# haotiansun14/rl-rep

Measured on NVIDIA B200. Metric: agent updates/sec, higher is better.
Workload: dtype tf32

## Files before the change

### rlrep_b200/csrc/gemm_chain.cu

```cuda
#include <algorithm>
#include <cmath>
#include <cstdlib>
#include <cstring>

#include "common.cuh"
#include "gemm_chain.cuh"
#include "ptx.cuh"

namespace rlrep {

namespace {

constexpr int kThreads = 320;
constexpr int kEpiWarps = 8;
constexpr int kStages = 6;
constexpr int kCW = 16;
constexpr int kTwPitch = kCW + 4;
constexpr int kMaxBn = 128;
constexpr int kBM = 128, kBK = 32;
constexpr int kABytes = kBM * kBK * 4;
constexpr int kStageBytes = kABytes + kMaxBn * kBK * 4;
constexpr int kTbufFloats = kEpiWarps * 32 * kTwPitch;
constexpr int kSub = 4, kCtrStride = 32;
constexpr int kDbgItems = 16, kDbgEvents = 10;
constexpr int kSmemBytes = kStages * kStageBytes + 1024 + 256 + kTbufFloats * 4;
static_assert(kSmemBytes <= 227 * 1024, "chain kernel shared memory");

__device__ __forceinline__ void red_release_add(unsigned* p, unsigned v) {
  asm volatile("red.release.gpu.global.add.u32 [%0], %1;" ::"l"(p), "r"(v) : "memory");
}
__device__ __forceinline__ unsigned atom_add_acq_rel(unsigned* p, unsigned v) {
  unsigned old;
  asm volatile("atom.acq_rel.gpu.global.add.u32 %0, [%1], %2;" : "=r"(old) : "l"(p), "r"(v) : "memory");
  return old;
}
__device__ __forceinline__ void fence_proxy_async_global() { asm volatile("fence.proxy.async.global;" ::: "memory"); }
__device__ __forceinline__ void fence_tensormap_acquire(const CUtensorMap* m) {
  asm volatile("fence.proxy.tensormap::generic.acquire.gpu [%0], 128;" ::"l"(reinterpret_cast<uint64_t>(m)) : "memory");
}
__device__ __forceinline__ unsigned ld_relaxed(const unsigned* p) {
  unsigned v;
  asm volatile("ld.relaxed.gpu.global.u32 %0, [%1];" : "=r"(v) : "l"(p) : "memory");
  return v;
}
__device__ __forceinline__ void wait_counter(const unsigned* done, int dep, int dep_tiles) {
  const unsigned* p = done + (size_t)dep * kSub * kCtrStride;
  unsigned target[kSub];
#pragma unroll
  for (int sub = 0; sub < kSub; ++sub) target[sub] = (unsigned)((dep_tiles - sub + kSub - 1) / kSub);
  long long t0 = 0;
  while (true) {
    unsigned v[kSub];
#pragma unroll
    for (int sub = 0; sub < kSub; ++sub) v[sub] = ld_relaxed(p + sub * kCtrStride);
    bool ok = true;
#pragma unroll
    for (int sub = 0; sub < kSub; ++sub) ok = ok && v[sub] >= target[sub];
    if (ok) return;
    __nanosleep(20);
    if (t0 == 0) t0 = clock64();
    if (clock64() - t0 > 4000000000LL) {
      printf("rlrep: chain dependency wait timed out (block %d, gemm %d, tiles %d, counters %u %u %u %u)\n", blockIdx.x, dep,
             dep_tiles, v[0], v[1], v[2], v[3]);
      __trap();
    }
  }
}
__device__ __forceinline__ void fence_acquire_gpu() { asm volatile("fence.acq_rel.gpu;" ::: "memory"); }

__device__ __forceinline__ void epilogue_bar() { asm volatile("bar.sync 1, 256;" ::: "memory"); }

__device__ __forceinline__ float elu_fast(float x) {
  const float n = fminf(x, 0.f);
  float p = 1.f / 5040.f;
  p = fmaf(p, n, 1.f / 720.f);
  p = fmaf(p, n, 1.f / 120.f);
  p = fmaf(p, n, 1.f / 24.f);
  p = fmaf(p, n, 1.f / 6.f);
  p = fmaf(p, n, 0.5f);
  p = fmaf(p, n, 1.f);
  p *= n;
  const float e = __expf(n) - 1.f;
  const float r = n < -0.34657359f ? e : p;
  return x > 0.f ? x : r;
}

__device__ __forceinline__ bool aligned16(const void* p) { return (reinterpret_cast<uintptr_t>(p) & 15) == 0; }

__device__ __forceinline__ float chain_epilogue_scalar(const Epilogue& e, float acc, int m, int n, const float* cptr) {
  float v = acc * e.scale;
  if (e.r1_u) v = fmaf(__ldcg(e.r1_u + m), __ldcg(e.r1_v + n), v);
  if (e.bias) v += __ldg(e.bias + n);
  if (e.pre_out) e.pre_out[(size_t)m * e.ld_pre + n] = v;
  v = apply_act(v, e.act);
  if (e.dact != DACT_NONE) v *= apply_dact(__ldcg(e.aux + (size_t)m * e.ld_aux + n), e.dact);
  if (e.accumulate) v += __ldcg(cptr);
  return v;
}

struct ChunkOperands {
  float4 bias, r1v;
  float4 aux[4];
  float r1u[4];
};
__device__ __forceinline__ void chunk_prefetch(ChunkOperands& o, const Epilogue& epi, int M, int m_base, int gn0, int lane) {
  const int piece = lane & 3, rsub = lane >> 2;
  const int on = gn0 + 4 * piece;
  o.bias = make_float4(0.f, 0.f, 0.f, 0.f);
  o.r1v = make_float4(0.f, 0.f, 0.f, 0.f);
  if (epi.bias) o.bias = __ldg(reinterpret_cast<const float4*>(epi.bias + on));
  if (epi.r1_u) o.r1v = __ldcg(reinterpret_cast<const float4*>(epi.r1_v + on));
#pragma unroll
  for (int r4 = 0; r4 < 4; ++r4) {
    const int om = m_base + r4 * 8 + rsub;
    o.aux[r4] = make_float4(0.f, 0.f, 0.f, 0.f);
    o.r1u[r4] = 0.f;
    if (om < M) {
      if (epi.dact != DACT_NONE) o.aux[r4] = __ldcg(reinterpret_cast<const float4*>(epi.aux + (size_t)om * epi.ld_aux + on));
      if (epi.r1_u) o.r1u[r4] = __ldcg(epi.r1_u + om);
    }
  }
}

template <int ACT, int DACT>
__device__ __forceinline__ void chain_store_rows(const Epilogue& epi, const ChunkOperands& o, const float* tw,
                                                 float* __restrict__ C, int ldc, int M, int m_base, int gn0, int lane) {
  const int piece = lane & 3, rsub = lane >> 2;
  const int on = gn0 + 4 * piece;
#pragma unroll
  for (int r4 = 0; r4 < 4; ++r4) {
    const int r = r4 * 8 + rsub;
    const int om = m_base + r;
    if (om < M) {
      const float4 a4 = *reinterpret_cast<const float4*>(tw + r * kTwPitch + 4 * piece);
      float v[4] = {a4.x * epi.scale, a4.y * epi.scale, a4.z * epi.scale, a4.w * epi.scale};
      if (epi.r1_u) {
        const float u = o.r1u[r4];
        v[0] = fmaf(u, o.r1v.x, v[0]); v[1] = fmaf(u, o.r1v.y, v[1]); v[2] = fmaf(u, o.r1v.z, v[2]); v[3] = fmaf(u, o.r1v.w, v[3]);
      }
      v[0] += o.bias.x; v[1] += o.bias.y; v[2] += o.bias.z; v[3] += o.bias.w;
      if (epi.pre_out)
        *reinterpret_cast<float4*>(epi.pre_out + (size_t)om * epi.ld_pre + on) = make_float4(v[0], v[1], v[2], v[3]);
      if constexpr (ACT != ACT_NONE) {
#pragma unroll
        for (int e = 0; e < 4; ++e) v[e] = ACT == ACT_ELU ? elu_fast(v[e]) : apply_act(v[e], ACT < 0 ? epi.act : ACT);
      }
      if constexpr (DACT != DACT_NONE) {
        const int dact = DACT < 0 ? epi.dact : DACT;
        if (dact != DACT_NONE) {
          const float4 x = o.aux[r4];
          v[0] *= apply_dact(x.x, dact); v[1] *= apply_dact(x.y, dact); v[2] *= apply_dact(x.z, dact); v[3] *= apply_dact(x.w, dact);
        }
      }
      float4* cp = reinterpret_cast<float4*>(C + (size_t)om * ldc + on);
      if (epi.accumulate) {
        const float4 c0 = __ldcg(cp);
        v[0] += c0.x; v[1] += c0.y; v[2] += c0.z; v[3] += c0.w;
      }
      *cp = make_float4(v[0], v[1], v[2], v[3]);
    }
  }
}

__global__ void __launch_bounds__(kThreads, 1)
gemm_chain_kernel(const ChainGemmDesc* __restrict__ gemms, const ChainTask* __restrict__ tasks,
                  const int* __restrict__ task_begin, unsigned* __restrict__ done, unsigned* __restrict__ exit_ctr,
                  int n_gemms, unsigned long long* __restrict__ dbg) {
  auto stamp = [&](int item, int ev) {
    if (dbg != nullptr && item < kDbgItems) {
      unsigned long long t;
      asm volatile("mov.u64 %0, %%globaltimer;" : "=l"(t)::"memory");
      dbg[((size_t)blockIdx.x * kDbgItems + item) * kDbgEvents + ev] = t;
    }
  };
  if (threadIdx.x == 0) stamp(kDbgItems - 1, 2);
  extern __shared__ uint8_t smem_raw[];
  uint8_t* smem = reinterpret_cast<uint8_t*>((reinterpret_cast<uintptr_t>(smem_raw) + 1023) & ~uintptr_t(1023));
  uint64_t* full_bar = reinterpret_cast<uint64_t*>(smem + kStages * kStageBytes);
  uint64_t* empty_bar = full_bar + 8;
  uint64_t* acc_full = empty_bar + 8;
  uint64_t* acc_empty = acc_full + 2;
  uint32_t* tmem_slot = reinterpret_cast<uint32_t*>(acc_empty + 2);
  volatile unsigned* arrival = reinterpret_cast<volatile unsigned*>(tmem_slot + 1);
  float* tbuf = reinterpret_cast<float*>(smem + kStages * kStageBytes + 256);

  const int warp = threadIdx.x >> 5, lane = threadIdx.x & 31;
  const int t_begin = task_begin[blockIdx.x], t_end = task_begin[blockIdx.x + 1];

  if (threadIdx.x == 0) {
    for (int s = 0; s < kStages; ++s) {
      ptx::mbar_init(&full_bar[s], 1);
      ptx::mbar_init(&empty_bar[s], 1);
    }
    for (int a = 0; a < 2; ++a) {
      ptx::mbar_init(&acc_full[a], 1);
      ptx::mbar_init(&acc_empty[a], kEpiWarps);
    }
    ptx::fence_mbar_init();
  }
  if (warp == 1) {
    ptx::tmem_alloc(tmem_slot, 2 * kMaxBn);
    ptx::tmem_relinquish();
  }
  ptx::tc_fence_before_sync();
  __syncthreads();
  ptx::tc_fence_after_sync();
  const uint32_t tmem_base = *tmem_slot;
  ptx::pdl_wait();

  if (warp == 0) {
    if (lane == 0) {
      int it = 0, last_gemm = -1;
      for (int t = t_begin; t < t_end; ++t) {
        const ChainTask tk = tasks[t];
        const ChainGemmDesc* g = gemms + tk.gemm;
        const int n_deps = g->n_deps;
        const int bn = g->bn, a_mn = g->a_mn, b_mn = g->b_mn;
        const int m0 = (tk.tile % g->tiles_m) * kBM, n0 = (tk.tile / g->tiles_m) * bn;
        const int kb0 = tk.split * g->kb_per_split, kb1 = min(g->nkb, kb0 + g->kb_per_split);
        int dep_id[kChainMaxDeps], dep_tiles[kChainMaxDeps];
#pragma unroll
        for (int d = 0; d < kChainMaxDeps; ++d) {
          dep_id[d] = d < n_deps ? g->dep[d] : 0;
          dep_tiles[d] = d < n_deps ? (int)g->dep_target[d] : 0;
        }
        if (tk.gemm != last_gemm) {
          fence_tensormap_acquire(&g->tmA);
          fence_tensormap_acquire(&g->tmB);
          last_gemm = tk.gemm;
        }
        stamp(t - t_begin, 0);
        if (dbg != nullptr && t - t_begin < kDbgItems)
          dbg[((size_t)blockIdx.x * kDbgItems + (t - t_begin)) * kDbgEvents + 8] =
              (unsigned long long)tk.gemm | ((unsigned long long)tk.tile << 16) | ((unsigned long long)tk.split << 40);
#pragma unroll
        for (int d = 0; d < kChainMaxDeps; ++d)
          if (d < n_deps) wait_counter(done, dep_id[d], dep_tiles[d]);
        if (n_deps > 0) {
          fence_acquire_gpu();
          fence_proxy_async_global();
        }
        stamp(t - t_begin, 1);
        const uint32_t tx = kABytes + bn * kBK * 4;
        for (int kb = kb0; kb < kb1; ++kb, ++it) {
          const int s = it % kStages;
          ptx::mbar_wait(&empty_bar[s], ((it / kStages) & 1) ^ 1);
          ptx::mbar_arrive_expect_tx(&full_bar[s], tx);
          uint8_t* a_dst = smem + s * kStageBytes;
          uint8_t* b_dst = a_dst + kABytes;
          const int k0 = kb * kBK;
          if (!a_mn) ptx::tma_load_2d(a_dst, &g->tmA, &full_bar[s], k0, m0);
          else ptx::tma_load_3d(a_dst, &g->tmA, &full_bar[s], 0, k0, m0 / 32);
          if (!b_mn) ptx::tma_load_2d(b_dst, &g->tmB, &full_bar[s], k0, n0);
          else ptx::tma_load_3d(b_dst, &g->tmB, &full_bar[s], 0, k0, n0 / 32);
        }
        stamp(t - t_begin, 2);
      }
    }
  } else if (warp == 1) {
    if (ptx::elect_one()) {
      int it = 0, tc = 0;
      for (int t = t_begin; t < t_end; ++t, ++tc) {
        const ChainTask tk = tasks[t];
        const ChainGemmDesc* g = gemms + tk.gemm;
        const int bn = g->bn, a_mn = g->a_mn, b_mn = g->b_mn;
        const int kb0 = tk.split * g->kb_per_split, kb1 = min(g->nkb, kb0 + g->kb_per_split);
        const uint32_t idesc = ptx::make_idesc_tf32(kBM, bn, a_mn != 0, b_mn != 0);
        const int acc = tc & 1;
        ptx::mbar_wait(&acc_empty[acc], ((tc >> 1) & 1) ^ 1);
        ptx::tc_fence_after_sync();
        const uint32_t d_tmem = tmem_base + acc * kMaxBn;
        for (int kb = kb0; kb < kb1; ++kb, ++it) {
          const int s = it % kStages;
          ptx::mbar_wait(&full_bar[s], (it / kStages) & 1);
          if (kb == kb0) stamp(t - t_begin, 3);
          ptx::tc_fence_after_sync();
          const uint32_t a_addr = ptx::smem_u32(smem + s * kStageBytes);
          const uint32_t b_addr = a_addr + kABytes;
#pragma unroll
          for (int k = 0; k < kBK / 8; ++k) {
            const uint64_t adesc = a_mn ? ptx::make_smem_desc(a_addr + k * 1024, 4096, 512, 1)
                                        : ptx::make_smem_desc(a_addr + k * 32, 16, 1024, 2);
            const uint64_t bdesc = b_mn ? ptx::make_smem_desc(b_addr + k * 1024, 4096, 512, 1)
                                        : ptx::make_smem_desc(b_addr + k * 32, 16, 1024, 2);
            ptx::mma_tf32_ss(d_tmem, adesc, bdesc, idesc, (kb > kb0 || k > 0) ? 1u : 0u);
          }
          ptx::mma_commit(&empty_bar[s]);
        }
        ptx::mma_commit(&acc_full[acc]);
        stamp(t - t_begin, 4);
      }
    }
  } else {
    const int q = warp & 3, half = (warp - 2) >> 2;
    float* tw = tbuf + (warp - 2) * (32 * kTwPitch);
    int tc = 0;
    for (int t = t_begin; t < t_end; ++t, ++tc) {
      const ChainTask tk = tasks[t];
      const ChainGemmDesc* g = gemms + tk.gemm;
      const Epilogue epi = g->epi;
      const int bn = g->bn, M = g->M, N = g->N, ldc = g->ldc, split_k = g->split_k;
      float* __restrict__ C = g->C;
      float* __restrict__ ws = g->ws;
      unsigned* __restrict__ tile_ctr = g->tile_ctr;
      const int m0 = (tk.tile % g->tiles_m) * kBM, n0 = (tk.tile / g->tiles_m) * bn;
      const int chunks = bn / kCW;
      const int acc = tc & 1;
      const uint32_t t_acc = tmem_base + (static_cast<uint32_t>(32 * q) << 16) + acc * kMaxBn;
      const int row = 32 * q + lane;
      ptx::mbar_wait(&acc_full[acc], (tc >> 1) & 1);
      if (threadIdx.x == 64) stamp(t - t_begin, 5);
      ptx::tc_fence_after_sync();

      bool final = true;
      const size_t part_floats = (size_t)kBM * bn;
      float* ws_tile = split_k > 1 ? ws + (size_t)tk.tile * split_k * part_floats : nullptr;
      const bool dist = split_k > 1 && g->dist != 0;
      int c_first = half, c_step = 2;
      if (split_k > 1) {
        float* part = ws_tile + (size_t)tk.split * part_floats;
#pragma unroll 1
        for (int c = half; c < chunks; c += 2) {
          if (dist && c % split_k == tk.split) continue;
          uint32_t v[kCW];
          ptx::tmem_ld_32x32b_x16(t_acc + c * kCW, v);
          ptx::tmem_ld_wait();
#pragma unroll
          for (int j = 0; j < kCW / 4; ++j)
            __stcg(reinterpret_cast<float4*>(part + ((size_t)(c * (kCW / 4) + j) * kBM + row) * 4),
                   make_float4(__uint_as_float(v[4 * j]), __uint_as_float(v[4 * j + 1]), __uint_as_float(v[4 * j + 2]),
                               __uint_as_float(v[4 * j + 3])));
        }
        epilogue_bar();
        if (threadIdx.x == 64) {
          unsigned* ctr = tile_ctr + tk.tile;
          const unsigned old = atom_add_acq_rel(ctr, 1u);
          if (dist) {
            if (old + 1 < (unsigned)split_k) {
              unsigned long long t0 = 0;
              unsigned spins = 0;
              while (ld_relaxed(ctr) < (unsigned)split_k) {
                __nanosleep(20);
                if ((++spins & 0xfff) == 0) {
                  unsigned long long now;
                  asm volatile("mov.u64 %0, %%globaltimer;" : "=l"(now));
                  if (t0 == 0) t0 = now;
                  else if (now - t0 > 2000000000ull) __trap();
                }
              }
              fence_acquire_gpu();
            }
          } else if (old == (unsigned)(split_k - 1)) {
            *ctr = 0;
          }
          *arrival = old;
          stamp(t - t_begin, 6);
        }
        epilogue_bar();
        final = dist || *arrival == (unsigned)(split_k - 1);
        if (dist) {
          c_first = tk.split + split_k * half;
          c_step = 2 * split_k;
        }
      }
      if (final) {
        const bool use_aux = epi.dact != DACT_NONE;
        const bool vec_ok = (ldc & 3) == 0 && aligned16(C) && (N & 3) == 0 &&
                            (!use_aux || ((epi.ld_aux & 3) == 0 && aligned16(epi.aux))) &&
                            (!epi.pre_out || ((epi.ld_pre & 3) == 0 && aligned16(epi.pre_out))) &&
                            (!epi.bias || aligned16(epi.bias)) && (!epi.r1_v || aligned16(epi.r1_v));
#pragma unroll 1
        for (int c = c_first; c < chunks; c += c_step) {
          const int gn0 = n0 + c * kCW;
          const bool fast = vec_ok && gn0 + kCW <= N;
          ChunkOperands ops;
          if (fast) chunk_prefetch(ops, epi, M, m0 + 32 * q, gn0, lane);
          float a[kCW];
          if (split_k == 1) {
            uint32_t v[kCW];
            ptx::tmem_ld_32x32b_x16(t_acc + c * kCW, v);
            ptx::tmem_ld_wait();
#pragma unroll
            for (int e = 0; e < kCW; ++e) a[e] = __uint_as_float(v[e]);
          } else {
            const float* base = ws_tile + ((size_t)(c * (kCW / 4)) * kBM + row) * 4;
            float4 nxt[kCW / 4];
            const int s_first = tk.split == 0 ? 1 : 0;
#pragma unroll
            for (int j = 0; j < kCW / 4; ++j)
              nxt[j] = __ldcg(reinterpret_cast<const float4*>(base + (size_t)s_first * part_floats + (size_t)j * kBM * 4));
#pragma unroll 1
            for (int s = 0; s < split_k; ++s) {
              if (s == tk.split) {
                uint32_t v[kCW];
                ptx::tmem_ld_32x32b_x16(t_acc + c * kCW, v);
                ptx::tmem_ld_wait();
                if (s == 0) {
#pragma unroll
                  for (int e = 0; e < kCW; ++e) a[e] = __uint_as_float(v[e]);
                } else {
#pragma unroll
                  for (int e = 0; e < kCW; ++e) a[e] += __uint_as_float(v[e]);
                }
                continue;
              }
              float4 cur[kCW / 4];
#pragma unroll
              for (int j = 0; j < kCW / 4; ++j) cur[j] = nxt[j];
              int s2 = s + 1;
              if (s2 == tk.split) ++s2;
              if (s2 < split_k) {
#pragma unroll
                for (int j = 0; j < kCW / 4; ++j)
                  nxt[j] = __ldcg(reinterpret_cast<const float4*>(base + (size_t)s2 * part_floats + (size_t)j * kBM * 4));
              }
              if (s == 0) {
#pragma unroll
                for (int j = 0; j < kCW / 4; ++j) { a[4 * j] = cur[j].x; a[4 * j + 1] = cur[j].y; a[4 * j + 2] = cur[j].z; a[4 * j + 3] = cur[j].w; }
              } else {
#pragma unroll
                for (int j = 0; j < kCW / 4; ++j) { a[4 * j] += cur[j].x; a[4 * j + 1] += cur[j].y; a[4 * j + 2] += cur[j].z; a[4 * j + 3] += cur[j].w; }
              }
            }
          }
#pragma unroll
          for (int j = 0; j < kCW / 4; ++j)
            *reinterpret_cast<float4*>(tw + lane * kTwPitch + 4 * j) = make_float4(a[4 * j], a[4 * j + 1], a[4 * j + 2], a[4 * j + 3]);
          __syncwarp();
          if (fast) {
#define RLREP_CSTORE(A, D) chain_store_rows<A, D>(epi, ops, tw, C, ldc, M, m0 + 32 * q, gn0, lane)
            RLREP_EPILOGUE_SWITCH(epi, RLREP_CSTORE);
#undef RLREP_CSTORE
          } else if (gn0 < N) {
            const int piece = lane & 3, rsub = lane >> 2;
#pragma unroll 1
            for (int r4 = 0; r4 < 4; ++r4) {
              const int r = r4 * 8 + rsub, om = m0 + 32 * q + r;
              if (om >= M) continue;
#pragma unroll 1
              for (int e = 0; e < 4; ++e) {
                const int on = gn0 + 4 * piece + e;
                if (on < N) {
                  float* cp = C + (size_t)om * ldc + on;
                  *cp = chain_epilogue_scalar(epi, tw[r * kTwPitch + 4 * piece + e], om, on, cp);
                }
              }
            }
          }
          __syncwarp();
        }
        if (threadIdx.x == 64) stamp(t - t_begin, 9);
        epilogue_bar();
        if (threadIdx.x == 64) {
          fence_proxy_async_global();
          const int pub = dist ? tk.tile * split_k + tk.split : tk.tile;
          red_release_add(done + ((size_t)tk.gemm * kSub + (pub % kSub)) * kCtrStride, 1u);
          stamp(t - t_begin, 7);
          if (dist) {
            unsigned* ctr = tile_ctr + tk.tile;
            if (atomicAdd(ctr, 1u) == (unsigned)(2 * split_k - 1)) *ctr = 0;
          }
        }
      }
      ptx::tc_fence_before_sync();
      __syncwarp();
      if (lane == 0) ptx::mbar_arrive(&acc_empty[acc]);
    }
  }
  ptx::pdl_launch_dependents();
  ptx::tc_fence_before_sync();
  __syncthreads();
  if (warp == 1) ptx::tmem_dealloc(tmem_base, 2 * kMaxBn);
  if (threadIdx.x == 0) {
    const unsigned old = atom_add_acq_rel(exit_ctr, 1u);
    if (old == gridDim.x - 1) {
      for (int i = 0; i < n_gemms * kSub; ++i) done[(size_t)i * kCtrStride] = 0;
      *exit_ctr = 0;
      __threadfence();
    }
    stamp(kDbgItems - 1, 3);
  }
}

struct Range {
  uintptr_t lo = 0, hi = 0;
  bool overlaps(const Range& o) const { return lo < o.hi && o.lo < hi && lo != hi && o.lo != o.hi; }
};
Range range_of(const float* p, long long rows, long long ld, long long cols) {
  Range r;
  if (p == nullptr || rows <= 0 || cols <= 0) return r;
  r.lo = reinterpret_cast<uintptr_t>(p);
  r.hi = r.lo + (size_t)((rows - 1) * ld + cols) * sizeof(float);
  return r;
}
struct Footprint {
  std::vector<Range> reads, writes;
};
Footprint footprint(const GemmArgs& a) {
  Footprint f;
  f.reads.push_back(a.a_mn ? range_of(a.A, a.K, a.lda, a.M) : range_of(a.A, a.M, a.lda, a.K));
  f.reads.push_back(a.b_mn ? range_of(a.B, a.K, a.ldb, a.N) : range_of(a.B, a.N, a.ldb, a.K));
  f.reads.push_back(range_of(a.epi.bias, 1, 0, a.N));
  f.reads.push_back(range_of(a.epi.r1_u, 1, 0, a.M));
  f.reads.push_back(range_of(a.epi.r1_v, 1, 0, a.N));
  if (a.epi.dact != DACT_NONE) f.reads.push_back(range_of(a.epi.aux, a.M, a.epi.ld_aux, a.N));
  f.writes.push_back(range_of(a.C, a.M, a.ldc, a.N));
  if (a.epi.accumulate) f.reads.push_back(f.writes.back());
  f.writes.push_back(range_of(a.epi.pre_out, a.M, a.epi.ld_pre, a.N));
  return f;
}
bool conflicts(const Footprint& earlier, const Footprint& later) {
  for (const Range& w : earlier.writes) {
    for (const Range& r : later.reads)
      if (w.overlaps(r)) return true;
    for (const Range& r : later.writes)
      if (w.overlaps(r)) return true;
  }
  for (const Range& w : later.writes)
    for (const Range& r : earlier.reads)
      if (w.overlaps(r)) return true;
  return false;
}

unsigned long long* g_chain_dbg = nullptr;

int env_int(const char* name, int dflt) {
  const char* e = std::getenv(name);
  return e ? std::atoi(e) : dflt;
}

bool dist_possible(int bn, int split) { return split > 1 && (bn / kCW) % split == 0; }
double plan_cost(int tiles, int nkb, int bn, int split, int share, bool dist) {
  const int kb_per = ceil_div(nkb, split);
  const double kb_bytes = kABytes + bn * kBK * 4;
  const double waves = std::ceil((double)tiles * split / share);
  const double stream = waves * kb_per * kb_bytes / 150e3;
  const double chip = (double)tiles * split * kb_per * kb_bytes / 12e6;
  if (dist) {
    return 1.5 + std::max(stream, chip) + waves * (0.25 * ceil_div(bn, 64) + 1.0 + 1.0 * ceil_div(bn / split, 64)) +
           0.1 * (split - 1);
  }
  double t = 1.5 + std::max(stream, chip) + waves * 1.0 * ceil_div(bn, 64);
  if (split > 1) t += 1.5 + 0.3 * (split - 1) * ceil_div(bn, 64);
  return t;
}

}

void set_chain_debug_buffer(unsigned long long* dev) { g_chain_dbg = dev; }

bool chain_eligible(const GemmArgs& a) {
  return tc_eligible(a) && a.conv_w == 0 && a.M >= 32 && a.N >= 32 && a.K >= 8;
}

GemmChain::~GemmChain() {
  if (dev_) cudaFree(dev_);
}

bool GemmChain::matches(const std::vector<GemmArgs>& seq) const {
  if (seq.size() != seq_.size()) return false;
  for (size_t i = 0; i < seq.size(); ++i) {
    const GemmArgs &x = seq[i], &y = seq_[i];
    if (x.M != y.M || x.N != y.N || x.K != y.K || x.A != y.A || x.B != y.B || x.C != y.C || x.lda != y.lda ||
        x.ldb != y.ldb || x.ldc != y.ldc || x.a_mn != y.a_mn || x.b_mn != y.b_mn || x.epi.bias != y.epi.bias ||
        x.epi.r1_u != y.epi.r1_u || x.epi.r1_v != y.epi.r1_v || x.epi.aux != y.epi.aux || x.epi.pre_out != y.epi.pre_out ||
        x.epi.ld_aux != y.epi.ld_aux || x.epi.ld_pre != y.epi.ld_pre || x.epi.act != y.epi.act || x.epi.dact != y.epi.dact ||
        x.epi.accumulate != y.epi.accumulate || x.epi.scale != y.epi.scale)
      return false;
  }
  return true;
}

void GemmChain::build(const std::vector<GemmArgs>& seq, int force_bn, int force_split) {
  RLREP_CHECK(dev_ == nullptr, "chain already built");
  RLREP_CHECK(!seq.empty(), "empty chain");
  const int n = (int)seq.size();
  for (const GemmArgs& a : seq) RLREP_CHECK(chain_eligible(a), "GEMM cannot be a member of a chain");
  seq_ = seq;
  int n_sm = kNumSMs;
  {
    int dev = 0;
    RLREP_CUDA(cudaGetDevice(&dev));
    RLREP_CUDA(cudaDeviceGetAttribute(&n_sm, cudaDevAttrMultiProcessorCount, dev));
  }
  static bool attr_set = false;
  if (!attr_set) {
    RLREP_CUDA(cudaFuncSetAttribute(gemm_chain_kernel, cudaFuncAttributeMaxDynamicSharedMemorySize, kSmemBytes));
    attr_set = true;
  }
  int per_sm = 0;
  RLREP_CUDA(cudaOccupancyMaxActiveBlocksPerMultiprocessor(&per_sm, gemm_chain_kernel, kThreads, kSmemBytes));
  RLREP_CHECK(per_sm >= 1, "chain kernel does not fit on an SM");
  const int n_cta = n_sm;

  std::vector<Footprint> fp(n);
  for (int i = 0; i < n; ++i) fp[i] = footprint(seq[i]);
  std::vector<std::vector<int>> deps(n);
  std::vector<std::vector<char>> reach(n, std::vector<char>(n, 0));
  std::vector<int> level(n, 0);
  for (int j = 0; j < n; ++j) {
    std::vector<int> direct;
    for (int i = 0; i < j; ++i)
      if (conflicts(fp[i], fp[j])) direct.push_back(i);
    for (int i : direct) {
      reach[j][i] = 1;
      for (int k = 0; k < n; ++k)
        if (reach[i][k]) reach[j][k] = 1;
    }
    for (int i : direct) {
      bool implied = false;
      for (int k : direct)
        if (k != i && reach[k][i]) implied = true;
      if (!implied) deps[j].push_back(i);
      level[j] = std::max(level[j], level[i] + 1);
    }
    RLREP_CHECK((int)deps[j].size() <= kChainMaxDeps, "a chain GEMM has too many direct dependencies");
  }
  levels_ = 1 + *std::max_element(level.begin(), level.end());

  std::vector<int> bn(n), split(n), share(n), first_cta(n), dist(n, 0);
  const int dist_mode = env_int("RLREP_CHAIN_DIST", 1);
  auto work_of = [&](int i) {
    return (double)ceil_div(seq[i].M, kBM) * ceil_div(seq[i].N, kMaxBn) * ceil_div(seq[i].K, kBK);
  };
  auto items_of = [&](int i) { return ceil_div(seq[i].M, kBM) * ceil_div(seq[i].N, bn[i]) * (dist[i] ? split[i] : 1); };
  for (int L = 0; L < levels_; ++L) {
    std::vector<int> members;
    for (int i = 0; i < n; ++i)
      if (level[i] == L) members.push_back(i);
    double total = 0.0;
    for (int i : members) total += work_of(i);
    int cursor = 0, seen = 0;
    for (int i : members) {
      const GemmArgs& a = seq[i];
      const int nkb = ceil_div(a.K, kBK);
      ++seen;
      int sh = std::max(4, (int)std::floor(n_cta * work_of(i) / total));
      if (seen == (int)members.size()) sh = std::max(sh, n_cta - cursor);
      sh = std::min(sh, n_cta);
      first_cta[i] = cursor % n_cta;
      cursor += sh;
      share[i] = sh;
      double best = 1e300;
      for (int cbn : {32, 64, 128}) {
        if (force_bn && cbn != force_bn) continue;
        if (!force_bn && cbn > 32 && cbn / 2 >= a.N) continue;
        const int tiles = ceil_div(a.M, kBM) * ceil_div(a.N, cbn);
        for (int s : {1, 2, 4, 8, 16}) {
          if (force_split && s != force_split) continue;
          if (s > 1 && (s - 1) * ceil_div(nkb, s) >= nkb) continue;
          for (int d = 0; d < 2; ++d) {
            if (d == 1 && (dist_mode == 0 || !dist_possible(cbn, s) || tiles * s > sh)) continue;
            if (d == 0 && dist_mode == 2 && dist_possible(cbn, s) && tiles * s <= sh) continue;
            const double c = plan_cost(tiles, nkb, cbn, s, sh, d == 1);
            if (c < best - 1e-9) {
              best = c;
              bn[i] = cbn;
              split[i] = s;
              dist[i] = d;
            }
          }
        }
      }
      if (best > 1e299) {
        bn[i] = force_bn ? force_bn : 32;
        split[i] = 1;
        dist[i] = 0;
      }
    }
  }

  std::vector<std::vector<ChainTask>> per_cta(n_cta);
  std::vector<int> order(n);
  for (int i = 0; i < n; ++i) order[i] = i;
  std::stable_sort(order.begin(), order.end(), [&](int x, int y) { return level[x] < level[y]; });
  size_t ws_floats = 0, ctr_count = 0;
  std::vector<size_t> ws_off(n, 0), ctr_off(n, 0);
  std::vector<ChainGemmDesc> descs(n);
  bytes_ = flops_ = 0.0;
  for (int i : order) {
    const GemmArgs& a = seq[i];
    const int tiles_m = ceil_div(a.M, kBM), tiles_n = ceil_div(a.N, bn[i]);
    const int tiles = tiles_m * tiles_n;
    int item = 0;
    for (int t = 0; t < tiles; ++t)
      for (int s = 0; s < split[i]; ++s, ++item)
        per_cta[(first_cta[i] + item % share[i]) % n_cta].push_back(ChainTask{i, t, s, 0});
    ChainGemmDesc& d = descs[i];
    std::memset(&d, 0, sizeof(d));
    d.tmA = make_operand_map(a.A, a.a_mn, a.M, a.K, a.lda, kBM);
    d.tmB = make_operand_map(a.B, a.b_mn, a.N, a.K, a.ldb, bn[i]);
    d.epi = a.epi;
    d.C = a.C;
    d.ldc = a.ldc; d.M = a.M; d.N = a.N; d.K = a.K;
    d.bn = bn[i]; d.a_mn = a.a_mn; d.b_mn = a.b_mn; d.nkb = ceil_div(a.K, kBK);
    d.split_k = split[i]; d.kb_per_split = ceil_div(d.nkb, split[i]);
    d.dist = dist[i];
    d.tiles_m = tiles_m; d.tiles_n = tiles_n;
    d.n_deps = (int)deps[i].size();
    for (int k = 0; k < d.n_deps; ++k) {
      const int j = deps[i][k];
      d.dep[k] = j;
      d.dep_target[k] = (unsigned)items_of(j);
    }
    ctr_off[i] = ctr_count;
    ctr_count += (size_t)tiles;
    if (split[i] > 1) {
      ws_off[i] = ws_floats;
      ws_floats += (size_t)tiles * split[i] * kBM * bn[i];
    }
    bytes_ += 4.0 * ((double)a.M * a.K + (double)a.N * a.K + (double)a.M * a.N);
    flops_ += 2.0 * a.M * a.N * a.K;
  }
  std::vector<ChainTask> tasks;
  std::vector<int> begin(n_cta + 1, 0);
  for (int c = 0; c < n_cta; ++c) {
    begin[c] = (int)tasks.size();
    tasks.insert(tasks.end(), per_cta[c].begin(), per_cta[c].end());
  }
  begin[n_cta] = (int)tasks.size();
  grid_ = n_cta;

  auto up = [](size_t x) { return (x + 255) & ~size_t(255); };
  const size_t o_desc = 0;
  const size_t o_tasks = up(o_desc + sizeof(ChainGemmDesc) * n);
  const size_t o_begin = up(o_tasks + sizeof(ChainTask) * tasks.size());
  const size_t o_done = up(o_begin + sizeof(int) * begin.size());
  const size_t o_exit = up(o_done + sizeof(unsigned) * n * kSub * kCtrStride);
  const size_t o_ctr = up(o_exit + sizeof(unsigned));
  const size_t o_ws = up(o_ctr + sizeof(unsigned) * ctr_count);
  const size_t total_bytes = o_ws + sizeof(float) * ws_floats + 256;
  RLREP_CUDA(cudaMalloc(&dev_, total_bytes));
  RLREP_CUDA(cudaMemset(dev_, 0, o_ws));
  char* base = static_cast<char*>(dev_);
  d_gemms_ = reinterpret_cast<ChainGemmDesc*>(base + o_desc);
  d_tasks_ = reinterpret_cast<ChainTask*>(base + o_tasks);
  d_task_begin_ = reinterpret_cast<int*>(base + o_begin);
  d_done_ = reinterpret_cast<unsigned*>(base + o_done);
  d_exit_ = reinterpret_cast<unsigned*>(base + o_exit);
  for (int i = 0; i < n; ++i) {
    descs[i].tile_ctr = reinterpret_cast<unsigned*>(base + o_ctr) + ctr_off[i];
    descs[i].ws = split[i] > 1 ? reinterpret_cast<float*>(base + o_ws) + ws_off[i] : nullptr;
  }
  RLREP_CUDA(cudaMemcpy(d_gemms_, descs.data(), sizeof(ChainGemmDesc) * n, cudaMemcpyHostToDevice));
  RLREP_CUDA(cudaMemcpy(d_tasks_, tasks.data(), sizeof(ChainTask) * tasks.size(), cudaMemcpyHostToDevice));
  RLREP_CUDA(cudaMemcpy(d_task_begin_, begin.data(), sizeof(int) * begin.size(), cudaMemcpyHostToDevice));
  RLREP_CUDA(cudaDeviceSynchronize());
  if (env_int("RLREP_CHAIN_VERBOSE", 0)) {
    std::fprintf(stderr, "rlrep chain: %d GEMMs, %d levels, %zu items, ws %.1f MB\n", n, levels_, tasks.size(),
                 ws_floats * 4 / 1e6);
    for (int i = 0; i < n; ++i)
      std::fprintf(stderr, "  [%d] L%d M=%d N=%d K=%d a_mn=%d b_mn=%d bn=%d split=%d%s share=%d deps=%d\n", i, level[i],
                   seq[i].M, seq[i].N, seq[i].K, (int)seq[i].a_mn, (int)seq[i].b_mn, bn[i], split[i],
                   dist[i] ? " (distributed)" : "", share[i], (int)deps[i].size());
  }
}

void GemmChain::launch(cudaStream_t stream) {
  RLREP_CHECK(dev_ != nullptr, "chain not built");
  cudaLaunchConfig_t cfg = {};
  cfg.gridDim = dim3(grid_);
  cfg.blockDim = dim3(kThreads);
  cfg.dynamicSmemBytes = kSmemBytes;
  cfg.stream = stream;
  cudaLaunchAttribute attr[2];
  attr[0].id = cudaLaunchAttributeCooperative;
  attr[0].val.cooperative = 1;
  attr[1] = pdl_attribute();
  cfg.attrs = attr;
  cfg.numAttrs = 2;
  RLREP_CUDA(cudaLaunchKernelEx(&cfg, gemm_chain_kernel, (const ChainGemmDesc*)d_gemms_, (const ChainTask*)d_tasks_,
                                (const int*)d_task_begin_, d_done_, d_exit_, (int)seq_.size(), g_chain_dbg));
  RLREP_LAUNCHED_W("gemm_chain", stream, bytes_, flops_);
}

}
```

### rlrep_b200/csrc/gemm_chain.cuh

```cuda
#pragma once
#include <vector>

#include "gemm.cuh"

namespace rlrep {

constexpr int kChainMaxDeps = 6;

struct alignas(128) ChainGemmDesc {
  CUtensorMap tmA;
  CUtensorMap tmB;
  Epilogue epi;
  int dist;
  float* C;
  float* ws;
  unsigned* tile_ctr;
  int ldc, M, N, K;
  int bn, a_mn, b_mn, nkb;
  int split_k, kb_per_split, tiles_m, tiles_n;
  int n_deps;
  int dep[kChainMaxDeps];
  unsigned dep_target[kChainMaxDeps];
};

struct ChainTask {
  int gemm, tile, split, pad;
};

class GemmChain {
 public:
  GemmChain() = default;
  GemmChain(const GemmChain&) = delete;
  GemmChain& operator=(const GemmChain&) = delete;
  ~GemmChain();
  bool matches(const std::vector<GemmArgs>& seq) const;
  void build(const std::vector<GemmArgs>& seq, int force_bn = 0, int force_split = 0);
  void launch(cudaStream_t stream);
  int size() const { return (int)seq_.size(); }
  int levels() const { return levels_; }

 private:
  std::vector<GemmArgs> seq_;
  void* dev_ = nullptr;
  ChainGemmDesc* d_gemms_ = nullptr;
  ChainTask* d_tasks_ = nullptr;
  int* d_task_begin_ = nullptr;
  unsigned* d_done_ = nullptr;
  unsigned* d_exit_ = nullptr;
  int grid_ = 0, levels_ = 0;
  double bytes_ = 0.0, flops_ = 0.0;
};

void set_chain_debug_buffer(unsigned long long* dev);

bool chain_eligible(const GemmArgs& a);

}
```

### rlrep_b200/csrc/ptx.cuh

```cuda
#pragma once
#include <cstdint>
#include <cuda.h>
#include <cuda_runtime.h>

namespace rlrep {
namespace ptx {

__device__ __forceinline__ uint32_t smem_u32(const void* p) {
  return static_cast<uint32_t>(__cvta_generic_to_shared(p));
}

__device__ __forceinline__ bool elect_one() {
  uint32_t pred = 0;
  asm volatile(
      "{\n"
      ".reg .b32 rx;\n"
      ".reg .pred px;\n"
      "elect.sync rx|px, 0xffffffff;\n"
      "selp.u32 %0, 1, 0, px;\n"
      "}\n"
      : "=r"(pred));
  return pred != 0;
}

__device__ __forceinline__ void pdl_wait() { asm volatile("griddepcontrol.wait;" ::: "memory"); }
__device__ __forceinline__ void pdl_launch_dependents() { asm volatile("griddepcontrol.launch_dependents;" ::: "memory"); }

__device__ __forceinline__ void mbar_init(uint64_t* bar, uint32_t count) {
  asm volatile("mbarrier.init.shared::cta.b64 [%0], %1;" ::"r"(smem_u32(bar)), "r"(count) : "memory");
}
__device__ __forceinline__ void fence_mbar_init() {
  asm volatile("fence.mbarrier_init.release.cluster;" ::: "memory");
}
__device__ __forceinline__ void fence_proxy_async_smem() {
  asm volatile("fence.proxy.async.shared::cta;" ::: "memory");
}
__device__ __forceinline__ void mbar_arrive_expect_tx(uint64_t* bar, uint32_t bytes) {
  asm volatile("mbarrier.arrive.expect_tx.shared::cta.b64 _, [%0], %1;" ::"r"(smem_u32(bar)), "r"(bytes)
               : "memory");
}
__device__ __forceinline__ void mbar_arrive(uint64_t* bar) {
  asm volatile("mbarrier.arrive.shared::cta.b64 _, [%0];" ::"r"(smem_u32(bar)) : "memory");
}
__device__ __forceinline__ bool mbar_try_wait(uint64_t* bar, uint32_t parity) {
  uint32_t ok;
  asm volatile(
      "{\n"
      ".reg .pred p;\n"
      "mbarrier.try_wait.parity.shared::cta.b64 p, [%1], %2;\n"
      "selp.u32 %0, 1, 0, p;\n"
      "}\n"
      : "=r"(ok)
      : "r"(smem_u32(bar)), "r"(parity)
      : "memory");
  return ok != 0;
}
__device__ __forceinline__ void mbar_wait(uint64_t* bar, uint32_t parity) {
  if (mbar_try_wait(bar, parity)) return;
  const long long t0 = clock64();
  while (!mbar_try_wait(bar, parity)) {
    if (clock64() - t0 > 4000000000LL) {
      printf("rlrep: mbarrier wait timed out (block %d,%d,%d thread %d)\n", blockIdx.x, blockIdx.y,
             blockIdx.z, threadIdx.x);
      __trap();
    }
  }
}

__device__ __forceinline__ void prefetch_tensormap(const CUtensorMap* m) {
  asm volatile("prefetch.tensormap [%0];" ::"l"(reinterpret_cast<uint64_t>(m)) : "memory");
}
__device__ __forceinline__ void tma_load_2d(void* smem_dst, const CUtensorMap* m, uint64_t* bar, int c_inner,
                                            int c_outer) {
  asm volatile(
      "cp.async.bulk.tensor.2d.shared::cluster.global.mbarrier::complete_tx::bytes [%0], [%1, {%3, %4}], [%2];"
      ::"r"(smem_u32(smem_dst)),
      "l"(reinterpret_cast<uint64_t>(m)), "r"(smem_u32(bar)), "r"(c_inner), "r"(c_outer)
      : "memory");
}
__device__ __forceinline__ void tma_load_3d(void* smem_dst, const CUtensorMap* m, uint64_t* bar, int c0, int c1, int c2) {
  asm volatile(
      "cp.async.bulk.tensor.3d.shared::cluster.global.mbarrier::complete_tx::bytes [%0], [%1, {%3, %4, %5}], [%2];"
      ::"r"(smem_u32(smem_dst)),
      "l"(reinterpret_cast<uint64_t>(m)), "r"(smem_u32(bar)), "r"(c0), "r"(c1), "r"(c2)
      : "memory");
}
__device__ __forceinline__ void tma_load_4d(void* smem_dst, const CUtensorMap* m, uint64_t* bar, int c0, int c1, int c2,
                                            int c3) {
  asm volatile(
      "cp.async.bulk.tensor.4d.shared::cluster.global.mbarrier::complete_tx::bytes [%0], [%1, {%3, %4, %5, %6}], [%2];"
      ::"r"(smem_u32(smem_dst)),
      "l"(reinterpret_cast<uint64_t>(m)), "r"(smem_u32(bar)), "r"(c0), "r"(c1), "r"(c2), "r"(c3)
      : "memory");
}
__device__ __forceinline__ void bulk_load_1d(void* smem_dst, const void* gsrc, uint32_t bytes, uint64_t* bar) {
  asm volatile(
      "cp.async.bulk.shared::cluster.global.mbarrier::complete_tx::bytes [%0], [%1], %2, [%3];" ::"r"(
          smem_u32(smem_dst)),
      "l"(reinterpret_cast<uint64_t>(gsrc)), "r"(bytes), "r"(smem_u32(bar))
      : "memory");
}

__device__ __forceinline__ void tmem_alloc(uint32_t* smem_result, uint32_t ncols) {
  asm volatile("tcgen05.alloc.cta_group::1.sync.aligned.shared::cta.b32 [%0], %1;" ::"r"(smem_u32(smem_result)),
               "r"(ncols)
               : "memory");
}
__device__ __forceinline__ void tmem_relinquish() {
  asm volatile("tcgen05.relinquish_alloc_permit.cta_group::1.sync.aligned;" ::: "memory");
}
__device__ __forceinline__ void tmem_dealloc(uint32_t taddr, uint32_t ncols) {
  asm volatile("tcgen05.dealloc.cta_group::1.sync.aligned.b32 %0, %1;" ::"r"(taddr), "r"(ncols) : "memory");
}
__device__ __forceinline__ void tc_fence_before_sync() {
  asm volatile("tcgen05.fence::before_thread_sync;" ::: "memory");
}
__device__ __forceinline__ void tc_fence_after_sync() {
  asm volatile("tcgen05.fence::after_thread_sync;" ::: "memory");
}
__device__ __forceinline__ void mma_tf32_ss(uint32_t tmem_d, uint64_t adesc, uint64_t bdesc, uint32_t idesc,
                                            uint32_t accumulate) {
  asm volatile(
      "{\n"
      ".reg .pred p;\n"
      "setp.ne.b32 p, %4, 0;\n"
      "tcgen05.mma.cta_group::1.kind::tf32 [%0], %1, %2, %3, p;\n"
      "}\n" ::"r"(tmem_d),
      "l"(adesc), "l"(bdesc), "r"(idesc), "r"(accumulate)
      : "memory");
}
__device__ __forceinline__ void mma_commit(uint64_t* bar) {
  asm volatile("tcgen05.commit.cta_group::1.mbarrier::arrive::one.shared::cluster.b64 [%0];" ::"r"(smem_u32(bar))
               : "memory");
}
__device__ __forceinline__ void tmem_ld_32x32b_x32(uint32_t taddr, uint32_t (&r)[32]) {
  asm volatile(
      "tcgen05.ld.sync.aligned.32x32b.x32.b32 "
      "{%0, %1, %2, %3, %4, %5, %6, %7, %8, %9, %10, %11, %12, %13, %14, %15, "
      "%16, %17, %18, %19, %20, %21, %22, %23, %24, %25, %26, %27, %28, %29, %30, %31}, [%32];"
      : "=r"(r[0]), "=r"(r[1]), "=r"(r[2]), "=r"(r[3]), "=r"(r[4]), "=r"(r[5]), "=r"(r[6]), "=r"(r[7]),
        "=r"(r[8]), "=r"(r[9]), "=r"(r[10]), "=r"(r[11]), "=r"(r[12]), "=r"(r[13]), "=r"(r[14]), "=r"(r[15]),
        "=r"(r[16]), "=r"(r[17]), "=r"(r[18]), "=r"(r[19]), "=r"(r[20]), "=r"(r[21]), "=r"(r[22]), "=r"(r[23]),
        "=r"(r[24]), "=r"(r[25]), "=r"(r[26]), "=r"(r[27]), "=r"(r[28]), "=r"(r[29]), "=r"(r[30]), "=r"(r[31])
      : "r"(taddr)
      : "memory");
}
__device__ __forceinline__ void tmem_ld_32x32b_x16(uint32_t taddr, uint32_t (&r)[16]) {
  asm volatile(
      "tcgen05.ld.sync.aligned.32x32b.x16.b32 "
      "{%0, %1, %2, %3, %4, %5, %6, %7, %8, %9, %10, %11, %12, %13, %14, %15}, [%16];"
      : "=r"(r[0]), "=r"(r[1]), "=r"(r[2]), "=r"(r[3]), "=r"(r[4]), "=r"(r[5]), "=r"(r[6]), "=r"(r[7]),
        "=r"(r[8]), "=r"(r[9]), "=r"(r[10]), "=r"(r[11]), "=r"(r[12]), "=r"(r[13]), "=r"(r[14]), "=r"(r[15])
      : "r"(taddr)
      : "memory");
}
__device__ __forceinline__ void tmem_ld_wait() { asm volatile("tcgen05.wait::ld.sync.aligned;" ::: "memory"); }

__device__ __forceinline__ void cluster_sync() {
  asm volatile("barrier.cluster.arrive.release.aligned;\n\tbarrier.cluster.wait.acquire.aligned;" ::: "memory");
}
__device__ __forceinline__ void cluster_arrive() {
  asm volatile("barrier.cluster.arrive.release.aligned;" ::: "memory");
}
__device__ __forceinline__ void cluster_arrive_relaxed() {
  asm volatile("barrier.cluster.arrive.relaxed.aligned;" ::: "memory");
}
__device__ __forceinline__ void cluster_wait() {
  asm volatile("barrier.cluster.wait.acquire.aligned;" ::: "memory");
}
__device__ __forceinline__ uint32_t cluster_ctarank() {
  uint32_t r;
  asm volatile("mov.u32 %0, %%cluster_ctarank;" : "=r"(r));
  return r;
}
__device__ __forceinline__ float4 ld_shared_f4(uint32_t addr) {
  float4 v;
  asm volatile("ld.shared.v4.f32 {%0, %1, %2, %3}, [%4];" : "=f"(v.x), "=f"(v.y), "=f"(v.z), "=f"(v.w) : "r"(addr) : "memory");
  return v;
}
__device__ __forceinline__ void st_dsmem_f4(uint32_t addr, uint32_t cta_rank, float4 v) {
  uint32_t remote;
  asm volatile("mapa.shared::cluster.u32 %0, %1, %2;" : "=r"(remote) : "r"(addr), "r"(cta_rank));
  asm volatile("st.shared::cluster.v4.f32 [%0], {%1, %2, %3, %4};" ::"r"(remote), "f"(v.x), "f"(v.y), "f"(v.z), "f"(v.w)
               : "memory");
}
__device__ __forceinline__ float4 ld_dsmem_f4(uint32_t addr, uint32_t cta_rank) {
  uint32_t remote;
  asm volatile("mapa.shared::cluster.u32 %0, %1, %2;" : "=r"(remote) : "r"(addr), "r"(cta_rank));
  float4 v;
  asm volatile("ld.shared::cluster.v4.f32 {%0, %1, %2, %3}, [%4];"
               : "=f"(v.x), "=f"(v.y), "=f"(v.z), "=f"(v.w)
               : "r"(remote)
               : "memory");
  return v;
}

__device__ __forceinline__ uint64_t make_smem_desc(uint32_t smem_addr, uint32_t lbo_bytes, uint32_t sbo_bytes,
                                                   uint32_t layout) {
  uint64_t d = 0;
  d |= static_cast<uint64_t>((smem_addr >> 4) & 0x3FFF);
  d |= static_cast<uint64_t>((lbo_bytes >> 4) & 0x3FFF) << 16;
  d |= static_cast<uint64_t>((sbo_bytes >> 4) & 0x3FFF) << 32;
  d |= static_cast<uint64_t>(1) << 46;
  d |= static_cast<uint64_t>(layout) << 61;
  return d;
}
__host__ __device__ constexpr uint32_t make_idesc_tf32(int m, int n, bool a_mn_major, bool b_mn_major) {
  return (1u << 4) | (2u << 7) | (2u << 10) | (static_cast<uint32_t>(a_mn_major) << 15) |
         (static_cast<uint32_t>(b_mn_major) << 16) | (static_cast<uint32_t>(n >> 3) << 17) |
         (static_cast<uint32_t>(m >> 4) << 24);
}

}
}
```

Measured before the change: 1308.

## Prefetch operands not produced in-chain before waiting on dependency counters

The producer warp now issues TMA loads for A/B operands that no earlier chain GEMM writes (e.g. weights), filling up to kStages stages before it blocks on the upstream dependency counters. Only the in-chain operand is loaded after the wait. This hides global-load latency behind inter-GEMM synchronisation. In exchange it adds host-side write/read overlap analysis, a split expect_tx accounting per stage, and some correctness risk in the mbarrier transaction bookkeeping.

After: 1315, median of 6. Within noise of the previous version (+0.6%).

```diff
diff --git a/rlrep_b200/csrc/gemm_chain.cu b/rlrep_b200/csrc/gemm_chain.cu
--- a/rlrep_b200/csrc/gemm_chain.cu
+++ b/rlrep_b200/csrc/gemm_chain.cu
@@ -233,6 +233,27 @@
         if (dbg != nullptr && t - t_begin < kDbgItems)
           dbg[((size_t)blockIdx.x * kDbgItems + (t - t_begin)) * kDbgEvents + 8] =
               (unsigned long long)tk.gemm | ((unsigned long long)tk.tile << 16) | ((unsigned long long)tk.split << 40);
+        auto load_a = [&](int s, int kb) {
+          uint8_t* dst = smem + s * kStageBytes;
+          if (!a_mn) ptx::tma_load_2d(dst, &g->tmA, &full_bar[s], kb * kBK, m0);
+          else ptx::tma_load_3d(dst, &g->tmA, &full_bar[s], 0, kb * kBK, m0 / 32);
+        };
+        auto load_b = [&](int s, int kb) {
+          uint8_t* dst = smem + s * kStageBytes + kABytes;
+          if (!b_mn) ptx::tma_load_2d(dst, &g->tmB, &full_bar[s], kb * kBK, n0);
+          else ptx::tma_load_3d(dst, &g->tmB, &full_bar[s], 0, kb * kBK, n0 / 32);
+        };
+        const uint32_t a_tx = kABytes, b_tx = bn * kBK * 4;
+        const bool pre_a = n_deps > 0 && !g->a_in_chain, pre_b = n_deps > 0 && !g->b_in_chain;
+        const int n_pre = (pre_a || pre_b) ? min(kb1 - kb0, kStages) : 0;
+        const uint32_t pre_tx = (pre_a ? a_tx : 0u) + (pre_b ? b_tx : 0u);
+        for (int i = 0; i < n_pre; ++i) {
+          const int s = (it + i) % kStages;
+          ptx::mbar_wait(&empty_bar[s], (((it + i) / kStages) & 1) ^ 1);
+          ptx::mbar_expect_tx(&full_bar[s], pre_tx);
+          if (pre_a) load_a(s, kb0 + i);
+          if (pre_b) load_b(s, kb0 + i);
+        }
 #pragma unroll
         for (int d = 0; d < kChainMaxDeps; ++d)
           if (d < n_deps) wait_counter(done, dep_id[d], dep_tiles[d]);
@@ -241,18 +262,13 @@
           fence_proxy_async_global();
         }
         stamp(t - t_begin, 1);
-        const uint32_t tx = kABytes + bn * kBK * 4;
         for (int kb = kb0; kb < kb1; ++kb, ++it) {
           const int s = it % kStages;
-          ptx::mbar_wait(&empty_bar[s], ((it / kStages) & 1) ^ 1);
-          ptx::mbar_arrive_expect_tx(&full_bar[s], tx);
-          uint8_t* a_dst = smem + s * kStageBytes;
-          uint8_t* b_dst = a_dst + kABytes;
-          const int k0 = kb * kBK;
-          if (!a_mn) ptx::tma_load_2d(a_dst, &g->tmA, &full_bar[s], k0, m0);
-          else ptx::tma_load_3d(a_dst, &g->tmA, &full_bar[s], 0, k0, m0 / 32);
-          if (!b_mn) ptx::tma_load_2d(b_dst, &g->tmB, &full_bar[s], k0, n0);
-          else ptx::tma_load_3d(b_dst, &g->tmB, &full_bar[s], 0, k0, n0 / 32);
+          const bool staged = kb - kb0 < n_pre;
+          if (!staged) ptx::mbar_wait(&empty_bar[s], ((it / kStages) & 1) ^ 1);
+          ptx::mbar_arrive_expect_tx(&full_bar[s], staged ? a_tx + b_tx - pre_tx : a_tx + b_tx);
+          if (!(staged && pre_a)) load_a(s, kb);
+          if (!(staged && pre_b)) load_b(s, kb);
         }
         stamp(t - t_begin, 2);
       }
@@ -616,6 +632,13 @@
     }
     RLREP_CHECK((int)deps[j].size() <= kChainMaxDeps, "a chain GEMM has too many direct dependencies");
   }
+  std::vector<char> a_in_chain(n, 0), b_in_chain(n, 0);
+  for (int j = 0; j < n; ++j)
+    for (int i = 0; i < j; ++i)
+      for (const Range& w : fp[i].writes) {
+        if (w.overlaps(fp[j].reads[0])) a_in_chain[j] = 1;
+        if (w.overlaps(fp[j].reads[1])) b_in_chain[j] = 1;
+      }
   levels_ = 1 + *std::max_element(level.begin(), level.end());
 
   std::vector<int> bn(n), split(n), share(n), first_cta(n), dist(n, 0);
@@ -698,6 +721,8 @@
     d.dist = dist[i];
     d.tiles_m = tiles_m; d.tiles_n = tiles_n;
     d.n_deps = (int)deps[i].size();
+    d.a_in_chain = a_in_chain[i];
+    d.b_in_chain = b_in_chain[i];
     for (int k = 0; k < d.n_deps; ++k) {
       const int j = deps[i][k];
       d.dep[k] = j;
@@ -750,9 +775,9 @@
     std::fprintf(stderr, "rlrep chain: %d GEMMs, %d levels, %zu items, ws %.1f MB\n", n, levels_, tasks.size(),
                  ws_floats * 4 / 1e6);
     for (int i = 0; i < n; ++i)
-      std::fprintf(stderr, "  [%d] L%d M=%d N=%d K=%d a_mn=%d b_mn=%d bn=%d split=%d%s share=%d deps=%d\n", i, level[i],
-                   seq[i].M, seq[i].N, seq[i].K, (int)seq[i].a_mn, (int)seq[i].b_mn, bn[i], split[i],
-                   dist[i] ? " (distributed)" : "", share[i], (int)deps[i].size());
+      std::fprintf(stderr, "  [%d] L%d M=%d N=%d K=%d a_mn=%d b_mn=%d bn=%d split=%d%s share=%d deps=%d in-chain A=%d B=%d\n",
+                   i, level[i], seq[i].M, seq[i].N, seq[i].K, (int)seq[i].a_mn, (int)seq[i].b_mn, bn[i], split[i],
+                   dist[i] ? " (distributed)" : "", share[i], (int)deps[i].size(), (int)a_in_chain[i], (int)b_in_chain[i]);
   }
 }
 
diff --git a/rlrep_b200/csrc/gemm_chain.cuh b/rlrep_b200/csrc/gemm_chain.cuh
--- a/rlrep_b200/csrc/gemm_chain.cuh
+++ b/rlrep_b200/csrc/gemm_chain.cuh
@@ -19,6 +19,7 @@
   int bn, a_mn, b_mn, nkb;
   int split_k, kb_per_split, tiles_m, tiles_n;
   int n_deps;
+  int a_in_chain, b_in_chain;
   int dep[kChainMaxDeps];
   unsigned dep_target[kChainMaxDeps];
 };
diff --git a/rlrep_b200/csrc/ptx.cuh b/rlrep_b200/csrc/ptx.cuh
--- a/rlrep_b200/csrc/ptx.cuh
+++ b/rlrep_b200/csrc/ptx.cuh
@@ -100,6 +100,9 @@
       "l"(reinterpret_cast<uint64_t>(gsrc)), "r"(bytes), "r"(smem_u32(bar))
       : "memory");
 }
+__device__ __forceinline__ void mbar_expect_tx(uint64_t* bar, uint32_t bytes) {
+  asm volatile("mbarrier.expect_tx.relaxed.cta.shared::cta.b64 [%0], %1;" ::"r"(smem_u32(bar)), "r"(bytes) : "memory");
+}
 
 __device__ __forceinline__ void tmem_alloc(uint32_t* smem_result, uint32_t ncols) {
   asm volatile("tcgen05.alloc.cta_group::1.sync.aligned.shared::cta.b32 [%0], %1;" ::"r"(smem_u32(smem_result)),
```
